# zdebruine/MMVAE

Hardware: AMD Instinct MI355X
Metric: cells/sec per MMVAE train step (higher is better)
Workload: dtype f32; 1 GPU; c2: 2-modality MMVAE train step, 20000 genes each, latent 128, K=1, batch 512/GPU, adversarial=False; global_batch=512, parallelism=dp1, exchange=none

## Files before the change

### include/mmvae_hip.h

```cpp
#ifndef MMVAE_HIP_H
#define MMVAE_HIP_H

#include <stddef.h>
#include <stdint.h>

#ifdef __cplusplus
extern "C" {
#endif

typedef void* mmvae_stream_t;

#define MMVAE_OK 0
#define MMVAE_ERR_ARG 1
#define MMVAE_ERR_LAUNCH 2
#define MMVAE_ERR_WORKSPACE 3

#define MMVAE_ABI_VERSION 13
int mmvae_abi_version(void);
const char* mmvae_build_arch(void);

#define MMVAE_GEMM_NT 0
#define MMVAE_GEMM_NN 1
#define MMVAE_GEMM_TN 2

#define MMVAE_GEMM_RELU 1u
#define MMVAE_GEMM_ACCUMULATE 2u
#define MMVAE_GEMM_RAW_SLABS 4u
#define MMVAE_GEMM_OPERAND_SLACK 8u

#define MMVAE_GEMM_PRECISION_F32 0
#define MMVAE_GEMM_PRECISION_BF16X3 1
int mmvae_gemm_set_precision(int mode);
int mmvae_gemm_set_workgroup_cap(int max_workgroups);
int mmvae_gemm_set_x3w(int mode);
int mmvae_gemm_get_x3w(void);
int mmvae_gemm_get_precision(void);

int mmvae_gemm_plan(int layout, int M, int N, int K, int* tile_out, int* splitk_out);
size_t mmvae_gemm_workspace_bytes(int layout, int M, int N, int K, int splitk);

int mmvae_gemm_f32(int layout, int M, int N, int K, float alpha, const float* A, int64_t lda, const float* B,
                   int64_t ldb, float* C, int64_t ldc, const float* bias, unsigned flags, int splitk,
                   float* workspace, size_t workspace_bytes, mmvae_stream_t stream);

int mmvae_recon_tiles(int G);
int mmvae_decoder_recon_f32(int B, int G, int H, const float* h, int64_t ldh, const float* W, int64_t ldw,
                            const float* bias, const float* x, int64_t ldx, float* xhat, int64_t ldxhat, float* dP,
                            int64_t lddp, float* se_part, mmvae_stream_t stream);
int mmvae_decoder_recon_rows_f32(int rows, int x_rows, int G, int H, const float* h, int64_t ldh, const float* W,
                                 int64_t ldw, const float* bias, const float* x, int64_t ldx, float* xhat,
                                 int64_t ldxhat, float* dP, int64_t lddp, float* se_part, mmvae_stream_t stream);
int mmvae_recon_set_h_kpad(int on);
int mmvae_recon_row_tiles(int rows);
int mmvae_decoder_recon_rows_colsum_f32(int rows, int x_rows, int G, int H, const float* h, int64_t ldh, const float* W,
                                        int64_t ldw, const float* bias, const float* x, int64_t ldx, float* xhat,
                                        int64_t ldxhat, float* dP, int64_t lddp, float* se_part, float* col_part,
                                        mmvae_stream_t stream);

typedef struct mmvae_bn_params {
    const float* gamma;
    const float* beta;
    float* running_mean;
    float* running_var;
    int64_t* num_batches_tracked;
    float momentum;
    float eps;
} mmvae_bn_params;

size_t mmvae_fc_workspace_bytes(int B, int N);

int mmvae_fc_epilogue_fwd(int B, int N, const float* in, int64_t ld_in, int n_slabs, const float* bias,
                          const mmvae_bn_params* bn , int training, int relu,
                          const uint8_t* keep_mask , float dropout_p, float* z_out,
                          float* a_out, float* d_out, int64_t ld_out, float* save_mean, float* save_invstd,
                          float* workspace, size_t workspace_bytes, mmvae_stream_t stream);

int mmvae_fc_epilogue_bwd(int B, int N, const float* din, int64_t ld_in, int n_slabs, const float* addend,
                          const float* addend_a, const float* row_scale, const uint8_t* keep_mask, float dropout_p, int relu,
                          const float* a, const float* z, const float* gamma, const float* save_mean,
                          const float* save_invstd, int has_bn, float* dz_out, int64_t ld_out, float* dbias,
                          float* dgamma, float* dbeta, float* workspace, size_t workspace_bytes,
                          mmvae_stream_t stream);

int mmvae_layernorm_fwd(int B, int N, const float* x, int64_t ldx, float eps, float* y, int64_t ldy, float* save_mean,
                        float* save_invstd, mmvae_stream_t stream);
int mmvae_layernorm_bwd(int B, int N, const float* dy, int64_t lddy, const float* y, int64_t ldy,
                        const float* save_invstd, float* dx, int64_t lddx, mmvae_stream_t stream);

int mmvae_fc_rowtail_fwd(int B, int N, const float* in, int64_t ld_in, int n_slabs, const float* bias ,
                         float eps, int training, int relu, const uint8_t* keep_mask , float dropout_p,
                         float* y_out, float* a_out, float* d_out, int64_t ld_out, float* save_invstd,
                         mmvae_stream_t stream);

int mmvae_fc_rowtail_bwd(int B, int N, const float* din, int64_t ld_in, int n_slabs, const float* addend,
                         const float* row_scale, const uint8_t* keep_mask, float dropout_p, int relu, const float* act,
                         const float* y, const float* save_invstd, float* dz_out, int64_t ld_out, float* dbias,
                         float* workspace, size_t workspace_bytes, mmvae_stream_t stream);

int mmvae_reparam_kl_fwd(int B, int Z, int K, const float* mu, const float* a_raw, const float* eps, float var_eps,
                         float* std_out, float* z_out, float* kl_row, float* stat_row, mmvae_stream_t stream);

int mmvae_reparam_kl_bwd(int B, int Z, int K, const float* mu, const float* std, const float* eps, const float* dz,
                         const float* dmu_extra, const float* dstd_extra, const float* dkl_row,
                         const float* kl_scale_dev, float kl_scale_host, float var_eps, float* dmu, float* da_raw,
                         mmvae_stream_t stream);

int mmvae_mse_sum_fwd_bwd(int B, int G, const float* xhat, int64_t ldxhat, const float* x, int64_t ldx, float* se_row,
                          float* dxhat, int64_t lddx, const float* gscale_dev, float gscale_host,
// ... 303 lines not shown
```

### mmvae_amd/_lib.py

```python
from __future__ import annotations

import ctypes as C
import os
from typing import Optional

_HERE = os.path.dirname(os.path.abspath(__file__))
LIB_PATH = os.path.join(_HERE, "csrc", "libmmvae_hip.so")
if os.environ.get("MMVAE_LIB"):
    LIB_PATH = os.environ["MMVAE_LIB"]

OK, ERR_ARG, ERR_LAUNCH, ERR_WORKSPACE = 0, 1, 2, 3
_ERR_NAMES = {1: "MMVAE_ERR_ARG", 2: "MMVAE_ERR_LAUNCH", 3: "MMVAE_ERR_WORKSPACE"}

GEMM_NT, GEMM_NN, GEMM_TN = 0, 1, 2
GEMM_RELU, GEMM_ACCUMULATE, GEMM_RAW_SLABS, GEMM_OPERAND_SLACK = 1, 2, 4, 8
GEMM_PRECISION_F32, GEMM_PRECISION_BF16X3 = 0, 1
ADAM_STATE_FLOATS = 8
ADAM_HYPER_FLOATS = 4
PREPARE_NORM, PREPARE_ADVANCE = 1, 2

_p = C.c_void_p
_i = C.c_int
_l = C.c_int64
_f = C.c_float
# ... 9 lines not shown
        ("beta", _p),
        ("running_mean", _p),
        ("running_var", _p),
        ("num_batches_tracked", _p),
        ("momentum", _f),
        ("eps", _f),
    ]


PROTOTYPES = {
    "mmvae_abi_version": (_i, []),
    "mmvae_build_arch": (C.c_char_p, []),
    "mmvae_gemm_set_precision": (_i, [_i]),
    "mmvae_gemm_set_workgroup_cap": (_i, [_i]),
    "mmvae_adam_set_workgroups": (_i, [_i]),
    "mmvae_recon_set_h_kpad": (_i, [_i]),
    "mmvae_adam_get_workgroups": (_i, []),
    "mmvae_gemm_set_x3w": (_i, [_i]),
    "mmvae_gemm_get_x3w": (_i, []),
    "mmvae_gemm_get_precision": (_i, []),
    "mmvae_gemm_plan": (_i, [_i, _i, _i, _i, C.POINTER(_i), C.POINTER(_i)]),
    "mmvae_gemm_workspace_bytes": (_z, [_i, _i, _i, _i, _i]),
    "mmvae_gemm_f32": (_i, [_i, _i, _i, _i, _f, _p, _l, _p, _l, _p, _l, _p, _u, _i, _p, _z, _p]),
    "mmvae_recon_tiles": (_i, [_i]),
    "mmvae_decoder_recon_f32": (_i, [_i, _i, _i, _p, _l, _p, _l, _p, _p, _l, _p, _l, _p, _l, _p, _p]),
    "mmvae_decoder_recon_rows_f32": (_i, [_i, _i, _i, _i, _p, _l, _p, _l, _p, _p, _l, _p, _l, _p, _l, _p, _p]),
    "mmvae_recon_row_tiles": (_i, [_i]),
    "mmvae_decoder_recon_rows_colsum_f32": (_i, [_i, _i, _i, _i, _p, _l, _p, _l, _p, _p, _l, _p, _l, _p, _l, _p, _p, _p]),
    "mmvae_fc_workspace_bytes": (_z, [_i, _i]),
    "mmvae_fc_epilogue_fwd": (
        _i,
        [_i, _i, _p, _l, _i, _p, C.POINTER(BnParams), _i, _i, _p, _f, _p, _p, _p, _l, _p, _p, _p, _z, _p],
    ),
    "mmvae_fc_epilogue_bwd": (
        _i,
        [_i, _i, _p, _l, _i, _p, _p, _p, _p, _f, _i, _p, _p, _p, _p, _p, _i, _p, _l, _p, _p, _p, _p, _z, _p],
    ),
    "mmvae_layernorm_fwd": (_i, [_i, _i, _p, _l, _f, _p, _l, _p, _p, _p]),
    "mmvae_layernorm_bwd": (_i, [_i, _i, _p, _l, _p, _l, _p, _p, _l, _p]),
    "mmvae_fc_rowtail_fwd": (_i, [_i, _i, _p, _l, _i, _p, _f, _i, _i, _p, _f, _p, _p, _p, _l, _p, _p]),
    "mmvae_fc_rowtail_bwd": (_i, [_i, _i, _p, _l, _i, _p, _p, _p, _f, _i, _p, _p, _p, _p, _l, _p, _p, _z, _p]),
    "mmvae_reparam_kl_fwd": (_i, [_i, _i, _i, _p, _p, _p, _f, _p, _p, _p, _p, _p]),
    "mmvae_reparam_kl_bwd": (_i, [_i, _i, _i, _p, _p, _p, _p, _p, _p, _p, _p, _f, _f, _p, _p, _p]),
    "mmvae_mse_sum_fwd_bwd": (_i, [_i, _i, _p, _l, _p, _l, _p, _p, _l, _p, _f, _p]),
    "mmvae_elbo_finalize": (_i, [_i, _i, _i, _p, _p, _p, _i, _p, _f, _p, _p, _p, _p]),
    "mmvae_iwae_logratio": (_i, [_i, _i, _i, _p, _p, _p, _p, _p]),
    "mmvae_elbo_finalize_iwae": (_i, [_i, _i, _i, _p, _p, _p, _i, _p, _f, _p, _p, _p, _p]),
    "mmvae_iwae_bwd_terms": (_i, [_i, _i, _i, _p, _f, _p, _p, _p, _p, _p, _p]),
    "mmvae_cross_entropy_sum": (_i, [_i, _i, _p, _l, _p, _p, _p, _l, _p, _f, _p]),
    "mmvae_cross_entropy_heads": (_i, [_i, _i, _i, _p, _p, _p, _l, _p, _p, _p, _l, _f, _p]),
    "mmvae_sum_f32": (_i, [_l, _p, _p, _i, _p]),
    "mmvae_debug_occupy": (_i, [_i, _i, _i, _p, _p]),
    "mmvae_sum_rows_f32": (_i, [_i, _l, _p, _l, _p, _p, _p]),
    "mmvae_sqnorm_partials": (_l, [_l]),
    "mmvae_grad_sqnorm": (_i, [_l, _p, _p, _p]),
    "mmvae_adam_prepare": (_i, [_l, _p, _f, _f, _f, _f, _p, _u, _p]),
    "mmvae_grad_sqnorm_ranges_prepare": (_i, [_i, _p, _p, _p, _p, _l, _p, _f, _f, _f, _f, _p, _u, _p]),
    "mmvae_adam_step": (_i, [_l, _p, _p, _p, _p, _p, _f, _f, _f, _f, _f, _f, _p]),
    "mmvae_adam_step_hp": (_i, [_l, _p, _p, _p, _p, _p, _p, _f, _f, _f, _f, _p]),
    "mmvae_adam_step_copy_hp": (_i, [_l, _p, _p, _p, _p, _p, _p, _f, _f, _f, _f, _i, _p, _p, _p]),
    "mmvae_adam_step_copy": (_i, [_l, _p, _p, _p, _p, _p, _f, _f, _f, _f, _f, _f, _i, _p, _p, _p]),
    "mmvae_adam_step_jobs": (_i, [_i, _p, _p, _p, _p, _p, _p, _f, _f, _f, _f, _f, _f, _p]),
    "mmvae_adam_step_jobs_hp": (_i, [_i, _p, _p, _p, _p, _p, _p, _p, _f, _f, _f, _f, _p]),
    "mmvae_grad_sqnorm_jobs": (_i, [_i, _p, _p, _p, _p]),
    "mmvae_grad_zero_flagged_jobs": (_i, [_i, _p, _p, _p]),
    "mmvae_jobs_pack": (_i, [_i, _p, _p, _p, _p]),
# ... 162 lines not shown
```

### mmvae_amd/csrc/fc_epilogue.hip

```cpp
#include "common.h"

namespace {

constexpr int CW = 64;
constexpr int RPC = 32;
constexpr int RPW = 8;
constexpr int CT = 256;

struct FwdArgs {
    const float* in;
    int64_t ld_in, slab_stride;
    int n_slabs;
    const float* bias;
    const float* gamma;
    const float* beta;
    float* running_mean;
    float* running_var;
    int64_t* nbt;
    float momentum, eps;
    int training, relu;
    const uint8_t* mask;
    float keep_scale;
    float* z_out;
    float* a_out;
// ... 13 lines not shown

__device__ __forceinline__ void split_rows_job(const FwdArgs& a, int wg, int nwg) {
    const int64_t total = (int64_t)a.sp_rows * a.sp_groups;
    for (int64_t idx = (int64_t)wg * CT + threadIdx.x; idx < total; idx += (int64_t)nwg * CT) {
        const int row = (int)(idx / a.sp_groups), gq = (int)(idx - (int64_t)row * a.sp_groups);
        const float* sp = a.sp_src + (int64_t)row * a.sp_ld_src + 8 * gq;
        f32x4 v0, v1;
        if (8 * gq + 8 <= a.sp_cols) {
            v0 = *reinterpret_cast<const f32x4*>(sp);
            v1 = *reinterpret_cast<const f32x4*>(sp + 4);
        } else {
            const int left = a.sp_cols - 8 * gq;
#pragma unroll
            for (int j = 0; j < 4; ++j) {
                v0[j] = j < left ? sp[j] : 0.f;
                v1[j] = 4 + j < left ? sp[4 + j] : 0.f;
            }
        }
        unsigned q[8][3];
#pragma unroll
        for (int j = 0; j < 4; ++j) {
            x3_split(v0[j], q[j][0], q[j][1], q[j][2]);
            x3_split(v1[j], q[4 + j][0], q[4 + j][1], q[4 + j][2]);
        }
        unsigned short* dp = a.sp_planes + (int64_t)row * a.sp_ld + 8 * gq;
#pragma unroll
        for (int p = 0; p < 3; ++p)
            *reinterpret_cast<uint4*>(dp + p * a.sp_pstride) =
                make_uint4((q[0][p] >> 16) | (q[1][p] & 0xFFFF0000u), (q[2][p] >> 16) | (q[3][p] & 0xFFFF0000u),
                           (q[4][p] >> 16) | (q[5][p] & 0xFFFF0000u), (q[6][p] >> 16) | (q[7][p] & 0xFFFF0000u));
    }
}

__device__ __forceinline__ float block_colsum(float v, float (*red)[CW], int w, int lane) {
    __syncthreads();
    red[w][lane] = v;
    __syncthreads();
    return (red[0][lane] + red[1][lane]) + (red[2][lane] + red[3][lane]);
}

__device__ __forceinline__ void slab_sum_rows(float (&acc)[RPW], const float* __restrict__ in, int64_t ld,
                                              int64_t slab_stride, int n_slabs, int r0, int B, int c) {
    const float* p[RPW];
#pragma unroll
    for (int i = 0; i < RPW; ++i) p[i] = in + (int64_t)min(r0 + i, B - 1) * ld + c;
    int s = 0;
    for (; s + 4 <= n_slabs; s += 4) {
        float t[4][RPW];
#pragma unroll
        for (int u = 0; u < 4; ++u)
#pragma unroll
            for (int i = 0; i < RPW; ++i) t[u][i] = p[i][(int64_t)(s + u) * slab_stride];
#pragma unroll
        for (int u = 0; u < 4; ++u)
#pragma unroll
            for (int i = 0; i < RPW; ++i) acc[i] += t[u][i];
    }
    for (; s < n_slabs; ++s) {
        float t[RPW];
#pragma unroll
        for (int i = 0; i < RPW; ++i) t[i] = p[i][(int64_t)s * slab_stride];
#pragma unroll
        for (int i = 0; i < RPW; ++i) acc[i] += t[i];
    }
}

__global__ __launch_bounds__(CT) void fc_fwd_stats_kernel(const FwdArgs a) {
    __shared__ float red[4][CW];
    const int lane = threadIdx.x & 63, w = threadIdx.x >> 6;
    const int c = blockIdx.x * CW + lane;
    const int chunk = blockIdx.y;
    const bool cv = c < a.N;
    const float bias = (cv && a.bias) ? a.bias[c] : 0.f;
    const int r0 = chunk * RPC + w * RPW;
    float zv[RPW];
    float s = 0.f;
#pragma unroll
    for (int i = 0; i < RPW; ++i) zv[i] = bias;
    slab_sum_rows(zv, a.in, a.ld_in, a.slab_stride, a.n_slabs, r0, a.B, cv ? c : a.N - 1);
#pragma unroll
    for (int i = 0; i < RPW; ++i) {
        const int r = r0 + i;
        if (cv && r < a.B) {
            a.z_out[(int64_t)r * a.ld_out + c] = zv[i];
            s += zv[i];
        } else {
            zv[i] = 0.f;
        }
    }
    const int nb = min(RPC, a.B - chunk * RPC);
    const float mean = block_colsum(s, red, w, lane) / (float)nb;
    float m2 = 0.f;
#pragma unroll
    for (int i = 0; i < RPW; ++i)
        if (r0 + i < a.B) {
            const float d = zv[i] - mean;
            m2 += d * d;
        }
    m2 = block_colsum(m2, red, w, lane);
    if (w == 0 && cv) {
        a.ws[(int64_t)chunk * a.N + c] = mean;
        a.ws[(int64_t)(a.RC + chunk) * a.N + c] = m2;
    }
}

template <bool HAS_BN>
__global__ __launch_bounds__(CT) void fc_fwd_apply_kernel(const FwdArgs a) {
    if ((int)blockIdx.y >= a.RC) {
        split_rows_job(a, ((int)blockIdx.y - a.RC) * gridDim.x + blockIdx.x, ((int)gridDim.y - a.RC) * gridDim.x);
        return;
    }
    const int lane = threadIdx.x & 63, w = threadIdx.x >> 6;
    const int c = blockIdx.x * CW + lane;
    const int chunk = blockIdx.y;
    if (c >= a.N) return;
    const float bias = a.bias ? a.bias[c] : 0.f;
    float mean = 0.f, invstd = 1.f, gam = 1.f, bet = 0.f;
    const bool stats = HAS_BN && a.training;
    const int r0 = chunk * RPC + w * RPW;
    float zs[RPW];
    unsigned char mk[RPW];
    if (stats || a.mask) {
#pragma unroll
        for (int i = 0; i < RPW; ++i) {
            const int rc = min(r0 + i, a.B - 1);
            if (stats) zs[i] = a.z_out[(int64_t)rc * a.ld_out + c];
            mk[i] = a.mask ? a.mask[(int64_t)rc * a.N + c] : (unsigned char)1;
        }
    }
    if (HAS_BN) {
        gam = a.gamma ? a.gamma[c] : 1.f;
        bet = a.beta ? a.beta[c] : 0.f;
        if (stats) {
            float n = 0.f, M2 = 0.f;
            for (int ch0 = 0; ch0 < a.RC; ch0 += 8) {
                float mb[8], m2b[8];
#pragma unroll
                for (int u = 0; u < 8; ++u) {
                    const int ch = min(ch0 + u, a.RC - 1);
                    mb[u] = a.ws[(int64_t)ch * a.N + c];
                    m2b[u] = a.ws[(int64_t)(a.RC + ch) * a.N + c];
                }
#pragma unroll
                for (int u = 0; u < 8; ++u) {
                    const int ch = ch0 + u;
                    if (ch < a.RC) {
                        const float nb = (float)min(RPC, a.B - ch * RPC);
                        const float delta = mb[u] - mean;
                        const float nn = n + nb;
                        mean += delta * (nb / nn);
                        M2 += m2b[u] + delta * delta * (n * nb / nn);
                        n = nn;
                    }
                }
            }
            const float var = M2 / (float)a.B;
            invstd = 1.0f / sqrtf(var + a.eps);
            if (chunk == 0 && w == 0) {
                if (a.save_mean) a.save_mean[c] = mean;
                if (a.save_invstd) a.save_invstd[c] = invstd;
                if (a.running_mean) a.running_mean[c] = (1.f - a.momentum) * a.running_mean[c] + a.momentum * mean;
                if (a.running_var) {
                    const float unb = a.B > 1 ? var * ((float)a.B / (float)(a.B - 1)) : var;
                    a.running_var[c] = (1.f - a.momentum) * a.running_var[c] + a.momentum * unb;
                }
                if (blockIdx.x == 0 && lane == 0 && a.nbt) *a.nbt += 1;
            }
        } else {
            mean = a.running_mean[c];
            invstd = 1.0f / sqrtf(a.running_var[c] + a.eps);
        }
    }
    if (!stats) {
#pragma unroll
        for (int i = 0; i < RPW; ++i) zs[i] = bias;
        slab_sum_rows(zs, a.in, a.ld_in, a.slab_stride, a.n_slabs, r0, a.B, c);
    }
#pragma unroll
    for (int i = 0; i < RPW; ++i) {
        const int r = r0 + i;
        if (r >= a.B) break;
        const int64_t o = (int64_t)r * a.ld_out + c;
        const float z = zs[i];
        if (!stats && a.z_out) a.z_out[o] = z;
        float y = z;
        if (HAS_BN) y = (z - mean) * invstd * gam + bet;
        if (a.relu) y = fmaxf(y, 0.f);
        if (a.a_out) a.a_out[o] = y;
        if (a.d_out) {
            float d = y;
            if (a.mask) d = mk[i] ? y * a.keep_scale : 0.f;
            a.d_out[o] = d;
            if (a.d_planes) store_planes_lanepair(a.d_planes, a.ldp, a.pstride, r, c, d, lane);
        }
    }
}

struct BwdArgs {
    const float* din;
    int64_t ld_in, slab_stride;
    int n_slabs;
    const float* addend;
    const float* addend_a;
    const float* row_scale;
    const uint8_t* mask;
    float keep_scale;
    int relu;
    const float* a;
    const float* z;
    const float* gamma;
    const float* save_mean;
    const float* save_invstd;
    float* dz_out;
    int64_t ld_out;
    float* dbias;
    float* dgamma;
    float* dbeta;
    float* ws;
    int B, N, RC;
    unsigned short* dz_planes;
    int64_t ldp, pstride;
};

struct BwdRowOps {
    float addend[RPW], row_scale[RPW], addend_a[RPW], act[RPW], z[RPW];
    unsigned char mask[RPW];
};
template <bool HAS_BN>
__device__ __forceinline__ void bwd_load_rows(const BwdArgs& a, int r0, int c, BwdRowOps& o) {
#pragma unroll
    for (int i = 0; i < RPW; ++i) {
        const int r = min(r0 + i, a.B - 1);
        const int64_t oo = (int64_t)r * a.ld_out + c;
        o.addend[i] = a.addend ? a.addend[oo] : 0.f;
        o.row_scale[i] = a.row_scale ? a.row_scale[r] : 1.f;
        o.mask[i] = a.mask ? a.mask[(int64_t)r * a.N + c] : (unsigned char)1;
        o.addend_a[i] = a.addend_a ? a.addend_a[oo] : 0.f;
        o.act[i] = a.relu ? a.a[oo] : 1.f;
        o.z[i] = HAS_BN ? a.z[oo] : 0.f;
    }
}
__device__ __forceinline__ float bwd_dy(const BwdArgs& a, const BwdRowOps& o, int i, float g) {
    if (a.addend) g += o.addend[i];
    if (a.row_scale) g *= o.row_scale[i];
    if (a.mask) g = o.mask[i] ? g * a.keep_scale : 0.f;
    if (a.addend_a) g += o.addend_a[i];
    if (a.relu) g = (o.act[i] > 0.f) ? g : 0.f;
    return g;
}

template <bool HAS_BN>
__global__ __launch_bounds__(CT) void fc_bwd_stats_kernel(const BwdArgs a) {
    __shared__ float red[4][CW];
    const int lane = threadIdx.x & 63, w = threadIdx.x >> 6;
    const int c = blockIdx.x * CW + lane;
    const int chunk = blockIdx.y;
    const bool cv = c < a.N;
    float mean = 0.f, invstd = 1.f;
    if (HAS_BN && cv) {
        mean = a.save_mean[c];
        invstd = a.save_invstd[c];
    }
    const int r0 = chunk * RPC + w * RPW;
    float s1 = 0.f, s2 = 0.f, s3 = 0.f;
    float gs[RPW];
#pragma unroll
    for (int i = 0; i < RPW; ++i) gs[i] = 0.f;
    BwdRowOps ops;
    bwd_load_rows<HAS_BN>(a, r0, cv ? c : a.N - 1, ops);
    slab_sum_rows(gs, a.din, a.ld_in, a.slab_stride, a.n_slabs, r0, a.B, cv ? c : a.N - 1);
#pragma unroll
    for (int i = 0; i < RPW; ++i) {
        const int r = r0 + i;
        if (cv && r < a.B) {
            const float dy = bwd_dy(a, ops, i, gs[i]);
            const int64_t oo = (int64_t)r * a.ld_out + c;
            if (a.dz_out) a.dz_out[oo] = dy;
            if (!HAS_BN && a.dz_planes) store_planes_lanepair(a.dz_planes, a.ldp, a.pstride, r, c, dy, lane);
            s1 += dy;
            if (HAS_BN) {
                const float xh = (ops.z[i] - mean) * invstd;
                s2 += dy * xh;
                s3 += xh;
            }
        }
    }
    if (!a.ws) return;
    s1 = block_colsum(s1, red, w, lane);
    if (HAS_BN) {
        s2 = block_colsum(s2, red, w, lane);
        s3 = block_colsum(s3, red, w, lane);
    }
    if (w == 0 && cv) {
        a.ws[(int64_t)chunk * a.N + c] = s1;
        if (HAS_BN) {
            a.ws[(int64_t)(a.RC + chunk) * a.N + c] = s2;
            a.ws[(int64_t)(2 * a.RC + chunk) * a.N + c] = s3;
        }
    }
}

__global__ __launch_bounds__(CT) void fc_bwd_apply_kernel(const BwdArgs a) {
    const int lane = threadIdx.x & 63, w = threadIdx.x >> 6;
    const int c = blockIdx.x * CW + lane;
    const int chunk = blockIdx.y;
    if (c >= a.N) return;
    const int r0 = chunk * RPC + w * RPW;
    float dys[RPW], zsv[RPW];
#pragma unroll
    for (int i = 0; i < RPW; ++i) {
        const int64_t oc = (int64_t)min(r0 + i, a.B - 1) * a.ld_out + c;
        dys[i] = a.dz_out[oc];
        zsv[i] = a.z[oc];
    }
    float S1 = 0.f, S2 = 0.f, S3 = 0.f;
    for (int ch0 = 0; ch0 < a.RC; ch0 += 8) {
        float t1[8], t2[8], t3[8];
#pragma unroll
        for (int u = 0; u < 8; ++u) {
            const int ch = min(ch0 + u, a.RC - 1);
            t1[u] = a.ws[(int64_t)ch * a.N + c];
            t2[u] = a.ws[(int64_t)(a.RC + ch) * a.N + c];
            t3[u] = a.ws[(int64_t)(2 * a.RC + ch) * a.N + c];
        }
#pragma unroll
        for (int u = 0; u < 8; ++u)
            if (ch0 + u < a.RC) {
                S1 += t1[u];
                S2 += t2[u];
                S3 += t3[u];
            }
    }
    const float mean = a.save_mean[c], invstd = a.save_invstd[c];
    const float gam = a.gamma ? a.gamma[c] : 1.f;
    const float invB = 1.f / (float)a.B;
    const float m1 = S1 * invB, m2 = S2 * invB;
    if (chunk == 0 && w == 0) {
        if (a.dbeta) a.dbeta[c] = S1;
        if (a.dgamma) a.dgamma[c] = S2;
        if (a.dbias) a.dbias[c] = -gam * invstd * m2 * S3;
    }
#pragma unroll
    for (int i = 0; i < RPW; ++i) {
        const int r = r0 + i;
        if (r >= a.B) break;
        const int64_t oo = (int64_t)r * a.ld_out + c;
        const float dy = dys[i];
        const float xh = (zsv[i] - mean) * invstd;
        const float dz = gam * invstd * (dy - m1 - xh * m2);
        a.dz_out[oo] = dz;
        if (a.dz_planes) store_planes_lanepair(a.dz_planes, a.ldp, a.pstride, r, c, dz, lane);
    }
}

__global__ __launch_bounds__(256) void fc_colsum_finish_kernel(const float* __restrict__ ws, int RC, int N,
                                                               float* __restrict__ dbias) {
    const int c = blockIdx.x * 256 + threadIdx.x;
    if (c >= N) return;
    float s = 0.f;
    for (int ch0 = 0; ch0 < RC; ch0 += 8) {
        float t[8];
#pragma unroll
        for (int u = 0; u < 8; ++u) t[u] = ws[(int64_t)min(ch0 + u, RC - 1) * N + c];
#pragma unroll
        for (int u = 0; u < 8; ++u)
            if (ch0 + u < RC) s += t[u];
    }
    dbias[c] = s;
}

__global__ __launch_bounds__(256) void layernorm_fwd_kernel(int B, int N, const float* __restrict__ x, int64_t ldx,
                                                            float eps, float* __restrict__ y, int64_t ldy,
                                                            float* save_mean, float* save_invstd) {
    const int lane = threadIdx.x & 63;
    const int row = blockIdx.x * 4 + (threadIdx.x >> 6);
    if (row >= B) return;
    const float* xr = x + (int64_t)row * ldx;
    float s = 0.f;
    for (int j = lane; j < N; j += 64) s += xr[j];
    const float mean = wave_sum(s) / (float)N;
    float s2 = 0.f;
    for (int j = lane; j < N; j += 64) {
        const float d = xr[j] - mean;
// ... 180 lines not shown
                a.dz_out[(int64_t)row * a.ld_out + c] = dz;
                col[k] += dz;
            }
        }
    }
    if (!a.ws) return;
#pragma unroll
    for (int k = 0; k < NV; ++k) red[w][lane + 64 * k] = col[k];
    __syncthreads();
    for (int c = threadIdx.x; c < a.N; c += 256)
        a.ws[(int64_t)chunk * a.N + c] = (red[0][c] + red[1][c]) + (red[2][c] + red[3][c]);
}

__global__ __launch_bounds__(256) void fc_rowtail_bwd_loop_kernel(const RowBwdArgs a) {
    const int lane = threadIdx.x & 63;
    const int row = blockIdx.x * 4 + (threadIdx.x >> 6);
    if (row >= a.B) return;
    const float rs = a.row_scale ? a.row_scale[row] : 1.f;
    const float* yr = a.y + (int64_t)row * a.ld_out;
    float* dr = a.dz_out + (int64_t)row * a.ld_out;
    float s1 = 0.f, s2 = 0.f;
    for (int c = lane; c < a.N; c += 64) {
        const float g = rowtail_dy(a, row, c, rs);
        dr[c] = g;
        s1 += g;
        s2 += g * yr[c];
    }
    const float m1 = wave_sum(s1) / (float)a.N, m2 = wave_sum(s2) / (float)a.N;
    const float invstd = a.save_invstd[row];
    for (int c = lane; c < a.N; c += 64) dr[c] = invstd * (dr[c] - m1 - yr[c] * m2);
}

}

extern "C" size_t mmvae_fc_workspace_bytes(int B, int N) {
    if (B <= 0 || N <= 0) return 0;
    return (size_t)3 * (size_t)ceil_div_i(B, RPC) * (size_t)N * sizeof(float);
}

static int fc_fwd_impl(int B, int N, const float* in, int64_t ld_in, int n_slabs, const float* bias,
                       const mmvae_bn_params* bn, int training, int relu, const uint8_t* keep_mask, float dropout_p,
                       float* z_out, float* a_out, float* d_out, int64_t ld_out, float* save_mean, float* save_invstd,
                       float* workspace, size_t workspace_bytes, uint16_t* d_planes, int64_t ldp, int64_t pstride,
                       mmvae_stream_t stream, int sp_rows = 0, int sp_cols = 0, const float* sp_src = nullptr,
                       int64_t sp_ld_src = 0, uint16_t* sp_planes = nullptr, int64_t sp_ld = 0, int64_t sp_pstride = 0) {
    if (d_planes && (!d_out || N % 2 != 0 || ldp < N || ldp % 2 != 0 || pstride < (int64_t)B * ldp)) return MMVAE_ERR_ARG;
    if (sp_planes && (sp_rows <= 0 || sp_cols <= 0 || !sp_src || sp_ld_src < sp_cols || sp_ld < (sp_cols + 7) / 8 * 8 ||
                      sp_ld % 8 != 0 || sp_pstride % 8 != 0 || sp_pstride < (int64_t)sp_rows * sp_ld ||
                      (reinterpret_cast<uintptr_t>(sp_planes) & 15u)))
        return MMVAE_ERR_ARG;
    if (B <= 0 || N <= 0 || !in || n_slabs < 1 || ld_in < N || ld_out < N) return MMVAE_ERR_ARG;
    if (!a_out && !d_out) return MMVAE_ERR_ARG;
    if (keep_mask && (dropout_p < 0.f || dropout_p >= 1.f || !d_out)) return MMVAE_ERR_ARG;
    if (bn && training && (!z_out || !save_mean || !save_invstd)) return MMVAE_ERR_ARG;
    if (bn && !training && (!bn->running_mean || !bn->running_var)) return MMVAE_ERR_ARG;
    const bool stats = bn && training;
    if (stats && (!workspace || workspace_bytes < mmvae_fc_workspace_bytes(B, N))) return MMVAE_ERR_WORKSPACE;
    FwdArgs a = {};
    a.in = in;
    a.ld_in = ld_in;
    a.slab_stride = (int64_t)B * ld_in;
    a.n_slabs = n_slabs;
    a.bias = bias;
    if (bn) {
        a.gamma = bn->gamma;
        a.beta = bn->beta;
// ... 4 lines not shown
        a.eps = bn->eps;
    }
    a.training = training;
    a.relu = relu;
    a.mask = keep_mask;
    a.keep_scale = keep_mask ? 1.0f / (1.0f - dropout_p) : 1.f;
    a.z_out = z_out;
    a.a_out = a_out;
    a.d_out = d_out;
    a.ld_out = ld_out;
    a.save_mean = save_mean;
    a.save_invstd = save_invstd;
    a.ws = workspace;
    a.B = B;
    a.N = N;
    a.RC = ceil_div_i(B, RPC);
    a.d_planes = reinterpret_cast<unsigned short*>(d_planes);
    a.ldp = ldp;
    a.pstride = pstride;
    const dim3 grid(ceil_div_i(N, CW), a.RC);
    dim3 grid_apply = grid;
    if (sp_planes) {
        a.sp_src = sp_src;
        a.sp_planes = reinterpret_cast<unsigned short*>(sp_planes);
        a.sp_ld_src = sp_ld_src;
        a.sp_ld = sp_ld;
        a.sp_pstride = sp_pstride;
        a.sp_rows = sp_rows;
        a.sp_groups = (sp_cols + 7) / 8;
        a.sp_cols = sp_cols;
        grid_apply.y = a.RC + ceil_div_i(768, (int)grid.x);
    }
    hipStream_t s = (hipStream_t)stream;
    if (stats) {
        MMVAE_LAUNCH(fc_fwd_stats_kernel, grid, dim3(CT), 0, s, a);
        MMVAE_LAUNCH_CHECK();
    }
    if (bn)
        MMVAE_LAUNCH(fc_fwd_apply_kernel<true>, grid_apply, dim3(CT), 0, s, a);
    else
        MMVAE_LAUNCH(fc_fwd_apply_kernel<false>, grid_apply, dim3(CT), 0, s, a);
    MMVAE_LAUNCH_CHECK();
    return MMVAE_OK;
}

extern "C" int mmvae_fc_epilogue_fwd(int B, int N, const float* in, int64_t ld_in, int n_slabs, const float* bias,
                                     const mmvae_bn_params* bn, int training, int relu, const uint8_t* keep_mask,
                                     float dropout_p, float* z_out, float* a_out, float* d_out, int64_t ld_out,
                                     float* save_mean, float* save_invstd, float* workspace, size_t workspace_bytes,
                                     mmvae_stream_t stream) {
    return fc_fwd_impl(B, N, in, ld_in, n_slabs, bias, bn, training, relu, keep_mask, dropout_p, z_out, a_out, d_out, ld_out,
                       save_mean, save_invstd, workspace, workspace_bytes, nullptr, 0, 0, stream);
}

extern "C" int mmvae_fc_epilogue_fwd_planes(int B, int N, const float* in, int64_t ld_in, int n_slabs, const float* bias,
                                            const mmvae_bn_params* bn, int training, int relu, const uint8_t* keep_mask,
                                            float dropout_p, float* z_out, float* a_out, float* d_out, int64_t ld_out,
                                            float* save_mean, float* save_invstd, float* workspace,
                                            size_t workspace_bytes, uint16_t* d_planes, int64_t ldp, int64_t plane_stride,
                                            mmvae_stream_t stream) {
    return fc_fwd_impl(B, N, in, ld_in, n_slabs, bias, bn, training, relu, keep_mask, dropout_p, z_out, a_out, d_out, ld_out,
                       save_mean, save_invstd, workspace, workspace_bytes, d_planes, ldp, plane_stride, stream);
}

extern "C" int mmvae_fc_epilogue_fwd_split(int B, int N, const float* in, int64_t ld_in, int n_slabs, const float* bias,
                                           const mmvae_bn_params* bn, int training, int relu, const uint8_t* keep_mask,
// ... 22 lines not shown
    if (!dz_out && !dbias && !workspace) return MMVAE_ERR_ARG;
    const bool need_ws = has_bn || dbias || workspace;
    if (need_ws && (!workspace || workspace_bytes < mmvae_fc_workspace_bytes(B, N))) return MMVAE_ERR_WORKSPACE;
    BwdArgs a = {};
    a.din = din;
    a.ld_in = ld_in;
    a.slab_stride = (int64_t)B * ld_in;
    a.n_slabs = n_slabs;
    a.addend = addend;
    a.addend_a = addend_a;
    a.row_scale = row_scale;
    a.mask = keep_mask;
    a.keep_scale = keep_mask ? 1.0f / (1.0f - dropout_p) : 1.f;
    a.relu = relu;
    a.a = a_act;
    a.z = z;
    a.gamma = gamma;
    a.save_mean = save_mean;
    a.save_invstd = save_invstd;
    a.dz_out = dz_out;
    a.ld_out = ld_out;
    a.dbias = dbias;
    a.dgamma = dgamma;
    a.dbeta = dbeta;
    a.ws = need_ws ? workspace : nullptr;
    a.B = B;
    a.N = N;
    a.RC = ceil_div_i(B, RPC);
    a.dz_planes = reinterpret_cast<unsigned short*>(dz_planes);
    a.ldp = ldp;
    a.pstride = pstride;
    const dim3 grid(ceil_div_i(N, CW), a.RC);
    hipStream_t s = (hipStream_t)stream;
    if (has_bn) {
        MMVAE_LAUNCH(fc_bwd_stats_kernel<true>, grid, dim3(CT), 0, s, a);
        MMVAE_LAUNCH_CHECK();
        MMVAE_LAUNCH(fc_bwd_apply_kernel, grid, dim3(CT), 0, s, a);
    } else {
        MMVAE_LAUNCH(fc_bwd_stats_kernel<false>, grid, dim3(CT), 0, s, a);
        MMVAE_LAUNCH_CHECK();
        if (dbias)
            MMVAE_LAUNCH(fc_colsum_finish_kernel, dim3(ceil_div_i(N, 256)), dim3(256), 0, s, workspace, a.RC, N,
                               dbias);
    }
    MMVAE_LAUNCH_CHECK();
    return MMVAE_OK;
}

extern "C" int mmvae_fc_epilogue_bwd(int B, int N, const float* din, int64_t ld_in, int n_slabs, const float* addend,
                                     const float* addend_a, const float* row_scale, const uint8_t* keep_mask, float dropout_p, int relu,
                                     const float* a_act, const float* z, const float* gamma, const float* save_mean,
                                     const float* save_invstd, int has_bn, float* dz_out, int64_t ld_out, float* dbias,
                                     float* dgamma, float* dbeta, float* workspace, size_t workspace_bytes,
                                     mmvae_stream_t stream) {
    return fc_bwd_impl(B, N, din, ld_in, n_slabs, addend, addend_a, row_scale, keep_mask, dropout_p, relu, a_act, z, gamma,
                       save_mean, save_invstd, has_bn, dz_out, ld_out, dbias, dgamma, dbeta, workspace, workspace_bytes,
                       nullptr, 0, 0, stream);
}

extern "C" int mmvae_fc_epilogue_bwd_planes(int B, int N, const float* din, int64_t ld_in, int n_slabs,
                                            const float* addend, const float* addend_a, const float* row_scale,
                                            const uint8_t* keep_mask, float dropout_p, int relu, const float* a_act,
                                            const float* z, const float* gamma, const float* save_mean,
                                            const float* save_invstd, int has_bn, float* dz_out, int64_t ld_out,
                                            float* dbias, float* dgamma, float* dbeta, float* workspace,
                                            size_t workspace_bytes, uint16_t* dz_planes, int64_t ldp,
                                            int64_t plane_stride, mmvae_stream_t stream) {
// ... 129 lines not shown
```

### mmvae_amd/ops.py

```python
from __future__ import annotations

import ctypes as C
from typing import Optional, Tuple

import torch

from . import _lib
from ._lib import GEMM_NT, GEMM_NN, GEMM_TN, GEMM_RELU, GEMM_ACCUMULATE, GEMM_RAW_SLABS

_workspaces: dict = {}


def _stream() -> int:
    return torch.cuda.current_stream().cuda_stream


def _chk(t: Optional[torch.Tensor], name: str, dtype=torch.float32) -> Optional[torch.Tensor]:
    if t is None:
        return None
    if not t.is_cuda:
        raise _lib.HipLibraryError(
            f"{name}: mmvae_amd HIP ops need a device tensor (got {t.device}); there is no CPU fallback. "
            "For CPU plumbing (BASELINE config C1) enable mmvae_amd.backend.cpu_plumbing()."
        )
# ... 299 lines not shown
        inp = inp.unsqueeze(0)
    if not inp.is_contiguous():
        raise ValueError("inp must be contiguous")
    S, B, N = inp.shape
    dev = inp.device
    has_drop = keep_mask is not None
    z = torch.empty((B, N), dtype=torch.float32, device=dev) if bn is not None else None
    d = torch.empty((B, N), dtype=torch.float32, device=dev)
    a = torch.empty((B, N), dtype=torch.float32, device=dev) if (has_drop and want_a) else None
    mean = invstd = None
    bnp = None
    if bn is not None:
        if training:
            mean = torch.empty(N, dtype=torch.float32, device=dev)
            invstd = torch.empty(N, dtype=torch.float32, device=dev)
        nbt = bn.get("num_batches_tracked")
        bnp = _lib.BnParams(
            _ptr(bn.get("gamma")), _ptr(bn.get("beta")), _ptr(bn.get("running_mean")), _ptr(bn.get("running_var")),
            _ptr(nbt) if nbt is not None else None, float(bn.get("momentum", 0.01)), float(bn.get("eps", 1e-3)),
        )
    if has_drop and (tuple(keep_mask.shape) != (B, N) or not keep_mask.is_contiguous()):
        raise ValueError("keep_mask must be contiguous [B,N] uint8")
    nws = lib.mmvae_fc_workspace_bytes(B, N)
    ws = workspace(nws, dev, "fc")
    rc = lib.mmvae_fc_epilogue_fwd(
        B, N, _ptr(inp), N, S, _ptr(bias), C.byref(bnp) if bnp is not None else None, int(training), int(relu),
        _ptr(keep_mask), float(dropout_p), _ptr(z), _ptr(a), _ptr(d), N, _ptr(mean), _ptr(invstd), _ptr(ws), nws,
        _stream(),
    )
    _lib.check(rc, "mmvae_fc_epilogue_fwd")
    return {"z": z, "a": a if a is not None else d, "d": d, "mean": mean, "invstd": invstd}


def fc_epilogue_bwd(
    din: torch.Tensor,
    *,
    addend: Optional[torch.Tensor] = None,
    addend_a: Optional[torch.Tensor] = None,
    row_scale: Optional[torch.Tensor] = None,
    keep_mask: Optional[torch.Tensor] = None,
    dropout_p: float = 0.0,
    relu: bool = False,
    a: Optional[torch.Tensor] = None,
    z: Optional[torch.Tensor] = None,
    gamma: Optional[torch.Tensor] = None,
    mean: Optional[torch.Tensor] = None,
    invstd: Optional[torch.Tensor] = None,
    has_bn: bool = False,
    want_dz: bool = True,
    want_dbias: bool = True,
    dbias_out: Optional[torch.Tensor] = None,
    dgamma_out: Optional[torch.Tensor] = None,
    dbeta_out: Optional[torch.Tensor] = None,
):
    lib = _lib.load()
    _chk(din, "din")
    if din.dim() == 2:
        din = din.unsqueeze(0)
    if not din.is_contiguous():
        raise ValueError("din must be contiguous")
    S, B, N = din.shape
    dev = din.device
    for name, t in (("addend", addend), ("addend_a", addend_a), ("a", a), ("z", z)):
        _chk(t, name)
        if t is not None and (tuple(t.shape) != (B, N) or not t.is_contiguous()):
            raise ValueError(f"{name} must be contiguous [B,N]")
# ... 490 lines not shown
```

Baseline: 577,400 cells/s.

## Fuse BN stats and apply into single-block-per-column-strip kernels for small batch

For batch sizes up to 512 with batchnorm, the FC epilogue forward and backward now run one kernel that holds all rows of a 16-column strip in one block. Each block reduces the column statistics through wavefront shuffles and shared memory, then applies the normalization, instead of running separate stats and apply launches that go through a global workspace. This removes a kernel launch and a workspace round trip per BN layer. In exchange, the grid is narrow-column with 1024-thread blocks, and the floating-point contraction order changes slightly. The path is on by default and can be switched off with an environment variable.

```diff
diff --git a/include/mmvae_hip.h b/include/mmvae_hip.h
--- a/include/mmvae_hip.h
+++ b/include/mmvae_hip.h
@@ -15,7 +15,7 @@
 #define MMVAE_ERR_LAUNCH 2
 #define MMVAE_ERR_WORKSPACE 3
 
-#define MMVAE_ABI_VERSION 13
+#define MMVAE_ABI_VERSION 14
 int mmvae_abi_version(void);
 const char* mmvae_build_arch(void);
 
@@ -74,6 +74,9 @@
                           const uint8_t* keep_mask , float dropout_p, float* z_out,
                           float* a_out, float* d_out, int64_t ld_out, float* save_mean, float* save_invstd,
                           float* workspace, size_t workspace_bytes, mmvae_stream_t stream);
+
+int mmvae_fc_set_fused_tail(int mode);
+int mmvae_fc_get_fused_tail(void);
 
 int mmvae_fc_epilogue_bwd(int B, int N, const float* din, int64_t ld_in, int n_slabs, const float* addend,
                           const float* addend_a, const float* row_scale, const uint8_t* keep_mask, float dropout_p, int relu,
diff --git a/mmvae_amd/_lib.py b/mmvae_amd/_lib.py
--- a/mmvae_amd/_lib.py
+++ b/mmvae_amd/_lib.py
@@ -65,6 +65,8 @@
         _i,
         [_i, _i, _p, _l, _i, _p, C.POINTER(BnParams), _i, _i, _p, _f, _p, _p, _p, _l, _p, _p, _p, _z, _p],
     ),
+    "mmvae_fc_set_fused_tail": (_i, [_i]),
+    "mmvae_fc_get_fused_tail": (_i, []),
     "mmvae_fc_epilogue_bwd": (
         _i,
         [_i, _i, _p, _l, _i, _p, _p, _p, _p, _f, _i, _p, _p, _p, _p, _p, _i, _p, _l, _p, _p, _p, _p, _z, _p],
diff --git a/mmvae_amd/csrc/fc_epilogue.hip b/mmvae_amd/csrc/fc_epilogue.hip
--- a/mmvae_amd/csrc/fc_epilogue.hip
+++ b/mmvae_amd/csrc/fc_epilogue.hip
@@ -69,27 +69,30 @@
     }
 }
 
+__device__ __forceinline__ float chunk_combine(float s0, float s1, float s2, float s3) { return (s0 + s1) + (s2 + s3); }
+
 __device__ __forceinline__ float block_colsum(float v, float (*red)[CW], int w, int lane) {
     __syncthreads();
     red[w][lane] = v;
     __syncthreads();
-    return (red[0][lane] + red[1][lane]) + (red[2][lane] + red[3][lane]);
-}
-
+    return chunk_combine(red[0][lane], red[1][lane], red[2][lane], red[3][lane]);
+}
+
+template <int SU = 4>
 __device__ __forceinline__ void slab_sum_rows(float (&acc)[RPW], const float* __restrict__ in, int64_t ld,
                                               int64_t slab_stride, int n_slabs, int r0, int B, int c) {
     const float* p[RPW];
 #pragma unroll
     for (int i = 0; i < RPW; ++i) p[i] = in + (int64_t)min(r0 + i, B - 1) * ld + c;
     int s = 0;
-    for (; s + 4 <= n_slabs; s += 4) {
-        float t[4][RPW];
-#pragma unroll
-        for (int u = 0; u < 4; ++u)
+    for (; s + SU <= n_slabs; s += SU) {
+        float t[SU][RPW];
+#pragma unroll
+        for (int u = 0; u < SU; ++u)
 #pragma unroll
             for (int i = 0; i < RPW; ++i) t[u][i] = p[i][(int64_t)(s + u) * slab_stride];
 #pragma unroll
-        for (int u = 0; u < 4; ++u)
+        for (int u = 0; u < SU; ++u)
 #pragma unroll
             for (int i = 0; i < RPW; ++i) acc[i] += t[u][i];
     }
@@ -99,6 +102,73 @@
         for (int i = 0; i < RPW; ++i) t[i] = p[i][(int64_t)s * slab_stride];
 #pragma unroll
         for (int i = 0; i < RPW; ++i) acc[i] += t[i];
+    }
+}
+
+
+__device__ __forceinline__ float fwd_store_z_sum(const FwdArgs& a, float (&zv)[RPW], int r0, int c, bool cv) {
+    float s = 0.f;
+#pragma unroll
+    for (int i = 0; i < RPW; ++i) {
+        const int r = r0 + i;
+        if (cv && r < a.B) {
+            a.z_out[(int64_t)r * a.ld_out + c] = zv[i];
+            s += zv[i];
+        } else {
+            zv[i] = 0.f;
+        }
+    }
+    return s;
+}
+__device__ __forceinline__ float fwd_m2_rows(const float (&zv)[RPW], int r0, int B, float mean) {
+#pragma clang fp contract(off)
+    float m2 = 0.f;
+#pragma unroll
+    for (int i = 0; i < RPW; ++i)
+        if (r0 + i < B) {
+            const float d = zv[i] - mean;
+            m2 = fmaf(d, d, m2);
+        }
+    return m2;
+}
+__device__ __forceinline__ void chan_merge(float& n, float& mean, float& M2, float nb, float mb, float m2b) {
+#pragma clang fp contract(off)
+    const float delta = mb - mean;
+    const float nn = n + nb;
+    mean += delta * (nb / nn);
+    M2 += fmaf(delta * delta, n * nb / nn, m2b);
+    n = nn;
+}
+__device__ __forceinline__ float fwd_finish_stats(const FwdArgs& a, int c, float mean, float M2, bool write, bool count) {
+#pragma clang fp contract(off)
+    const float var = M2 / (float)a.B;
+    const float invstd = 1.0f / sqrtf(var + a.eps);
+    if (write) {
+        if (a.save_mean) a.save_mean[c] = mean;
+        if (a.save_invstd) a.save_invstd[c] = invstd;
+        if (a.running_mean) a.running_mean[c] = (1.f - a.momentum) * a.running_mean[c] + a.momentum * mean;
+        if (a.running_var) {
+            const float unb = a.B > 1 ? var * ((float)a.B / (float)(a.B - 1)) : var;
+            a.running_var[c] = (1.f - a.momentum) * a.running_var[c] + a.momentum * unb;
+        }
+        if (count && a.nbt) *a.nbt += 1;
+    }
+    return invstd;
+}
+template <bool HAS_BN>
+__device__ __forceinline__ void fwd_apply_elem(const FwdArgs& a, int r, int c, int lane, float z, unsigned char mk,
+                                               float mean, float invstd, float gam, float bet) {
+#pragma clang fp contract(off)
+    const int64_t o = (int64_t)r * a.ld_out + c;
+    float y = z;
+    if (HAS_BN) y = fmaf((z - mean) * invstd, gam, bet);
+    if (a.relu) y = fmaxf(y, 0.f);
+    if (a.a_out) a.a_out[o] = y;
+    if (a.d_out) {
+        float d = y;
+        if (a.mask) d = mk ? y * a.keep_scale : 0.f;
+        a.d_out[o] = d;
+        if (a.d_planes) store_planes_lanepair(a.d_planes, a.ldp, a.pstride, r, c, d, lane);
     }
 }
 
@@ -111,30 +181,13 @@
     const float bias = (cv && a.bias) ? a.bias[c] : 0.f;
     const int r0 = chunk * RPC + w * RPW;
     float zv[RPW];
-    float s = 0.f;
 #pragma unroll
     for (int i = 0; i < RPW; ++i) zv[i] = bias;
     slab_sum_rows(zv, a.in, a.ld_in, a.slab_stride, a.n_slabs, r0, a.B, cv ? c : a.N - 1);
-#pragma unroll
-    for (int i = 0; i < RPW; ++i) {
-        const int r = r0 + i;
-        if (cv && r < a.B) {
-            a.z_out[(int64_t)r * a.ld_out + c] = zv[i];
-            s += zv[i];
-        } else {
-            zv[i] = 0.f;
-        }
-    }
+    const float s = fwd_store_z_sum(a, zv, r0, c, cv);
     const int nb = min(RPC, a.B - chunk * RPC);
     const float mean = block_colsum(s, red, w, lane) / (float)nb;
-    float m2 = 0.f;
-#pragma unroll
-    for (int i = 0; i < RPW; ++i)
-        if (r0 + i < a.B) {
-            const float d = zv[i] - mean;
-            m2 += d * d;
-        }
-    m2 = block_colsum(m2, red, w, lane);
+    const float m2 = block_colsum(fwd_m2_rows(zv, r0, a.B, mean), red, w, lane);
     if (w == 0 && cv) {
         a.ws[(int64_t)chunk * a.N + c] = mean;
         a.ws[(int64_t)(a.RC + chunk) * a.N + c] = m2;
@@ -181,28 +234,10 @@
 #pragma unroll
                 for (int u = 0; u < 8; ++u) {
                     const int ch = ch0 + u;
-                    if (ch < a.RC) {
-                        const float nb = (float)min(RPC, a.B - ch * RPC);
-                        const float delta = mb[u] - mean;
-                        const float nn = n + nb;
-                        mean += delta * (nb / nn);
-                        M2 += m2b[u] + delta * delta * (n * nb / nn);
-                        n = nn;
-                    }
+                    if (ch < a.RC) chan_merge(n, mean, M2, (float)min(RPC, a.B - ch * RPC), mb[u], m2b[u]);
                 }
             }
-            const float var = M2 / (float)a.B;
-            invstd = 1.0f / sqrtf(var + a.eps);
-            if (chunk == 0 && w == 0) {
-                if (a.save_mean) a.save_mean[c] = mean;
-                if (a.save_invstd) a.save_invstd[c] = invstd;
-                if (a.running_mean) a.running_mean[c] = (1.f - a.momentum) * a.running_mean[c] + a.momentum * mean;
-                if (a.running_var) {
-                    const float unb = a.B > 1 ? var * ((float)a.B / (float)(a.B - 1)) : var;
-                    a.running_var[c] = (1.f - a.momentum) * a.running_var[c] + a.momentum * unb;
-                }
-                if (blockIdx.x == 0 && lane == 0 && a.nbt) *a.nbt += 1;
-            }
+            invstd = fwd_finish_stats(a, c, mean, M2, chunk == 0 && w == 0, blockIdx.x == 0 && lane == 0);
         } else {
             mean = a.running_mean[c];
             invstd = 1.0f / sqrtf(a.running_var[c] + a.eps);
@@ -217,19 +252,8 @@
     for (int i = 0; i < RPW; ++i) {
         const int r = r0 + i;
         if (r >= a.B) break;
-        const int64_t o = (int64_t)r * a.ld_out + c;
-        const float z = zs[i];
-        if (!stats && a.z_out) a.z_out[o] = z;
-        float y = z;
-        if (HAS_BN) y = (z - mean) * invstd * gam + bet;
-        if (a.relu) y = fmaxf(y, 0.f);
-        if (a.a_out) a.a_out[o] = y;
-        if (a.d_out) {
-            float d = y;
-            if (a.mask) d = mk[i] ? y * a.keep_scale : 0.f;
-            a.d_out[o] = d;
-            if (a.d_planes) store_planes_lanepair(a.d_planes, a.ldp, a.pstride, r, c, d, lane);
-        }
+        if (!stats && a.z_out) a.z_out[(int64_t)r * a.ld_out + c] = zs[i];
+        fwd_apply_elem<HAS_BN>(a, r, c, lane, zs[i], mk[i], mean, invstd, gam, bet);
     }
 }
 
@@ -278,12 +302,39 @@
     }
 }
 __device__ __forceinline__ float bwd_dy(const BwdArgs& a, const BwdRowOps& o, int i, float g) {
+#pragma clang fp contract(off)
     if (a.addend) g += o.addend[i];
     if (a.row_scale) g *= o.row_scale[i];
     if (a.mask) g = o.mask[i] ? g * a.keep_scale : 0.f;
     if (a.addend_a) g += o.addend_a[i];
     if (a.relu) g = (o.act[i] > 0.f) ? g : 0.f;
     return g;
+}
+
+__device__ __forceinline__ float bn_xhat(float z, float mean, float invstd) { return (z - mean) * invstd; }
+template <bool HAS_BN>
+__device__ __forceinline__ void bwd_acc(float dy, float z, float mean, float invstd, float& s1, float& s2, float& s3) {
+#pragma clang fp contract(off)
+    s1 += dy;
+    if (HAS_BN) {
+        const float xh = bn_xhat(z, mean, invstd);
+        s2 += dy * xh;
+        s3 += xh;
+    }
+}
+__device__ __forceinline__ float bwd_dz(float gam, float invstd, float dy, float z, float mean, float S1, float invB,
+                                        float m2, bool first) {
+#pragma clang fp contract(off)
+    const float xh = bn_xhat(z, mean, invstd);
+    const float t = first ? fmaf(-invB, S1, dy) : dy - S1 * invB;
+    return gam * invstd * fmaf(-m2, xh, t);
+}
+__device__ __forceinline__ void bwd_col_outputs(const BwdArgs& a, int c, float gam, float invstd, float m2, float S1,
+                                                float S2, float S3) {
+#pragma clang fp contract(off)
+    if (a.dbeta) a.dbeta[c] = S1;
+    if (a.dgamma) a.dgamma[c] = S2;
+    if (a.dbias) a.dbias[c] = -gam * invstd * m2 * S3;
 }
 
 template <bool HAS_BN>
@@ -314,12 +365,7 @@
             const int64_t oo = (int64_t)r * a.ld_out + c;
             if (a.dz_out) a.dz_out[oo] = dy;
             if (!HAS_BN && a.dz_planes) store_planes_lanepair(a.dz_planes, a.ldp, a.pstride, r, c, dy, lane);
-            s1 += dy;
-            if (HAS_BN) {
-                const float xh = (ops.z[i] - mean) * invstd;
-                s2 += dy * xh;
-                s3 += xh;
-            }
+            bwd_acc<HAS_BN>(dy, ops.z[i], mean, invstd, s1, s2, s3);
         }
     }
     if (!a.ws) return;
@@ -371,21 +417,131 @@
     const float mean = a.save_mean[c], invstd = a.save_invstd[c];
     const float gam = a.gamma ? a.gamma[c] : 1.f;
     const float invB = 1.f / (float)a.B;
-    const float m1 = S1 * invB, m2 = S2 * invB;
-    if (chunk == 0 && w == 0) {
-        if (a.dbeta) a.dbeta[c] = S1;
-        if (a.dgamma) a.dgamma[c] = S2;
-        if (a.dbias) a.dbias[c] = -gam * invstd * m2 * S3;
-    }
+    const float m2 = S2 * invB;
+    if (chunk == 0 && w == 0) bwd_col_outputs(a, c, gam, invstd, m2, S1, S2, S3);
 #pragma unroll
     for (int i = 0; i < RPW; ++i) {
         const int r = r0 + i;
         if (r >= a.B) break;
         const int64_t oo = (int64_t)r * a.ld_out + c;
-        const float dy = dys[i];
-        const float xh = (zsv[i] - mean) * invstd;
-        const float dz = gam * invstd * (dy - m1 - xh * m2);
+        const float dz = bwd_dz(gam, invstd, dys[i], zsv[i], mean, S1, invB, m2, i == 0);
         a.dz_out[oo] = dz;
+        if (a.dz_planes) store_planes_lanepair(a.dz_planes, a.ldp, a.pstride, r, c, dz, lane);
+    }
+}
+
+constexpr int FROWS = 512;
+constexpr int FSUB = FROWS / RPW;
+constexpr int FCH = FROWS / RPC;
+
+template <int SW>
+__device__ __forceinline__ float chunk_sum_lanes(float v, int base) {
+    const float s0 = __shfl(v, base, 64), s1 = __shfl(v, base + SW, 64);
+    const float s2 = __shfl(v, base + 2 * SW, 64), s3 = __shfl(v, base + 3 * SW, 64);
+    return chunk_combine(s0, s1, s2, s3);
+}
+
+template <int SW>
+__global__ __launch_bounds__(FSUB * SW) void fc_fwd_fused_kernel(const FwdArgs a) {
+    static_assert(64 % (4 * SW) == 0 && SW % 2 == 0, "a chunk's sub-chunks share a wavefront, lane pairs a row");
+    __shared__ float pmean[FCH][SW], pm2[FCH][SW];
+    const int lane = threadIdx.x & 63;
+    const int col = threadIdx.x % SW, sub = threadIdx.x / SW;
+    const int c = blockIdx.x * SW + col;
+    const bool cv = c < a.N;
+    const int cc = cv ? c : a.N - 1;
+    const int chunk = sub >> 2;
+    const int r0 = sub * RPW;
+    const int base = lane - (sub & 3) * SW;
+    unsigned char mk[RPW];
+#pragma unroll
+    for (int i = 0; i < RPW; ++i)
+        mk[i] = a.mask ? a.mask[(int64_t)min(r0 + i, a.B - 1) * a.N + cc] : (unsigned char)1;
+    const float bias = a.bias ? a.bias[cc] : 0.f;
+    const float gam = a.gamma ? a.gamma[cc] : 1.f, bet = a.beta ? a.beta[cc] : 0.f;
+    float zv[RPW];
+#pragma unroll
+    for (int i = 0; i < RPW; ++i) zv[i] = bias;
+    slab_sum_rows<2>(zv, a.in, a.ld_in, a.slab_stride, a.n_slabs, r0, a.B, cc);
+    const float s = fwd_store_z_sum(a, zv, r0, c, cv);
+    const int nb = max(min(RPC, a.B - chunk * RPC), 1);
+    const float cmean = chunk_sum_lanes<SW>(s, base) / (float)nb;
+    const float cm2 = chunk_sum_lanes<SW>(fwd_m2_rows(zv, r0, a.B, cmean), base);
+    if ((sub & 3) == 0) {
+        pmean[chunk][col] = cmean;
+        pm2[chunk][col] = cm2;
+    }
+    __syncthreads();
+    float n = 0.f, mean = 0.f, M2 = 0.f;
+    for (int ch = 0; ch < a.RC; ++ch) chan_merge(n, mean, M2, (float)min(RPC, a.B - ch * RPC), pmean[ch][col], pm2[ch][col]);
+    const float invstd = fwd_finish_stats(a, c, mean, M2, cv && sub == 0, blockIdx.x == 0 && threadIdx.x == 0);
+    if (!cv) return;
+#pragma unroll
+    for (int i = 0; i < RPW; ++i) {
+        const int r = r0 + i;
+        if (r >= a.B) break;
+        fwd_apply_elem<true>(a, r, c, lane, zv[i], mk[i], mean, invstd, gam, bet);
+    }
+}
+
+template <int SW>
+__global__ __launch_bounds__(FSUB * SW) void fc_bwd_fused_kernel(const BwdArgs a) {
+    static_assert(64 % (4 * SW) == 0 && SW % 2 == 0, "a chunk's sub-chunks share a wavefront, lane pairs a row");
+    __shared__ float part[3][FCH][SW];
+    const int lane = threadIdx.x & 63;
+    const int col = threadIdx.x % SW, sub = threadIdx.x / SW;
+    const int c = blockIdx.x * SW + col;
+    const bool cv = c < a.N;
+    const int cc = cv ? c : a.N - 1;
+    const int chunk = sub >> 2;
+    const int r0 = sub * RPW;
+    const int base = lane - (sub & 3) * SW;
+    const float mean = a.save_mean[cc], invstd = a.save_invstd[cc];
+    const float gam = a.gamma ? a.gamma[cc] : 1.f;
+    float dys[RPW], zs[RPW];
+    float s1 = 0.f, s2 = 0.f, s3 = 0.f;
+    {
+        float gs[RPW];
+#pragma unroll
+        for (int i = 0; i < RPW; ++i) gs[i] = 0.f;
+        slab_sum_rows<2>(gs, a.din, a.ld_in, a.slab_stride, a.n_slabs, r0, a.B, cc);
+        BwdRowOps ops;
+        bwd_load_rows<true>(a, r0, cc, ops);
+#pragma unroll
+        for (int i = 0; i < RPW; ++i) {
+            zs[i] = ops.z[i];
+            dys[i] = 0.f;
+            if (cv && r0 + i < a.B) {
+                dys[i] = bwd_dy(a, ops, i, gs[i]);
+                bwd_acc<true>(dys[i], zs[i], mean, invstd, s1, s2, s3);
+            }
+        }
+    }
+    s1 = chunk_sum_lanes<SW>(s1, base);
+    s2 = chunk_sum_lanes<SW>(s2, base);
+    s3 = chunk_sum_lanes<SW>(s3, base);
+    if ((sub & 3) == 0) {
+        part[0][chunk][col] = s1;
+        part[1][chunk][col] = s2;
+        part[2][chunk][col] = s3;
+    }
+    __syncthreads();
+    float S1 = 0.f, S2 = 0.f, S3 = 0.f;
+    for (int ch = 0; ch < a.RC; ++ch) {
+        S1 += part[0][ch][col];
+        S2 += part[1][ch][col];
+        S3 += part[2][ch][col];
+    }
+    if (!cv) return;
+    const float invB = 1.f / (float)a.B;
+    const float m2 = S2 * invB;
+    if (sub == 0) bwd_col_outputs(a, c, gam, invstd, m2, S1, S2, S3);
+#pragma unroll
+    for (int i = 0; i < RPW; ++i) {
+        const int r = r0 + i;
+        if (r >= a.B) break;
+        const float dz = bwd_dz(gam, invstd, dys[i], zs[i], mean, S1, invB, m2, i == 0);
+        a.dz_out[(int64_t)r * a.ld_out + c] = dz;
         if (a.dz_planes) store_planes_lanepair(a.dz_planes, a.ldp, a.pstride, r, c, dz, lane);
     }
 }
@@ -632,6 +788,27 @@
 }
 
 }
+
+static int g_fused_tail = -1;
+static constexpr bool FUSED_TAIL_DEFAULT = true;
+#ifndef FC_FUSED_SW8_MAX_N
+#define FC_FUSED_SW8_MAX_N 0
+#endif
+static bool fused_narrow_strip(int N) { return N <= FC_FUSED_SW8_MAX_N; }
+static bool fused_tail_enabled() {
+    if (g_fused_tail >= 0) return g_fused_tail != 0;
+    const char* e = getenv("MMVAE_FC_FUSED_TAIL");
+    if (!e || !e[0]) return FUSED_TAIL_DEFAULT;
+    return e[0] != '0';
+}
+
+extern "C" int mmvae_fc_set_fused_tail(int mode) {
+    if (mode < -1 || mode > 1) return MMVAE_ERR_ARG;
+    g_fused_tail = mode;
+    return MMVAE_OK;
+}
+
+extern "C" int mmvae_fc_get_fused_tail(void) { return g_fused_tail; }
 
 extern "C" size_t mmvae_fc_workspace_bytes(int B, int N) {
     if (B <= 0 || N <= 0) return 0;
@@ -702,6 +879,14 @@
         grid_apply.y = a.RC + ceil_div_i(768, (int)grid.x);
     }
     hipStream_t s = (hipStream_t)stream;
+    if (stats && B <= FROWS && !sp_planes && fused_tail_enabled()) {
+        if (fused_narrow_strip(N))
+            MMVAE_LAUNCH(fc_fwd_fused_kernel<8>, dim3(ceil_div_i(N, 8)), dim3(FSUB * 8), 0, s, a);
+        else
+            MMVAE_LAUNCH(fc_fwd_fused_kernel<16>, dim3(ceil_div_i(N, 16)), dim3(FSUB * 16), 0, s, a);
+        MMVAE_LAUNCH_CHECK();
+        return MMVAE_OK;
+    }
     if (stats) {
         MMVAE_LAUNCH(fc_fwd_stats_kernel, grid, dim3(CT), 0, s, a);
         MMVAE_LAUNCH_CHECK();
@@ -790,7 +975,12 @@
     a.pstride = pstride;
     const dim3 grid(ceil_div_i(N, CW), a.RC);
     hipStream_t s = (hipStream_t)stream;
-    if (has_bn) {
+    if (has_bn && B <= FROWS && fused_tail_enabled()) {
+        if (fused_narrow_strip(N))
+            MMVAE_LAUNCH(fc_bwd_fused_kernel<8>, dim3(ceil_div_i(N, 8)), dim3(FSUB * 8), 0, s, a);
+        else
+            MMVAE_LAUNCH(fc_bwd_fused_kernel<16>, dim3(ceil_div_i(N, 16)), dim3(FSUB * 16), 0, s, a);
+    } else if (has_bn) {
         MMVAE_LAUNCH(fc_bwd_stats_kernel<true>, grid, dim3(CT), 0, s, a);
         MMVAE_LAUNCH_CHECK();
         MMVAE_LAUNCH(fc_bwd_apply_kernel, grid, dim3(CT), 0, s, a);
diff --git a/mmvae_amd/ops.py b/mmvae_amd/ops.py
--- a/mmvae_amd/ops.py
+++ b/mmvae_amd/ops.py
@@ -355,6 +355,14 @@
     return {"z": z, "a": a if a is not None else d, "d": d, "mean": mean, "invstd": invstd}
 
 
+def fc_set_fused_tail(mode: int) -> None:
+    _lib.check(_lib.load().mmvae_fc_set_fused_tail(int(mode)), "mmvae_fc_set_fused_tail")
+
+
+def fc_get_fused_tail() -> int:
+    return _lib.load().mmvae_fc_get_fused_tail()
+
+
 def fc_epilogue_bwd(
     din: torch.Tensor,
     *,
```

Result: no change. 573,700 cells/s (median of 2 runs) (-0.6%).
